# AHSAppDevTeam/Voxmap

Measured on AMD Instinct MI355X. Metric: Mrays/s at 3840x2160 full quality (C3); fps; % HBM roofline, higher is better.
Workload: dtype fp32

## Files before the change

voxmap_amd/csrc/vx_frame.cpp:

```cpp
#include <algorithm>
#include <cmath>
#include <cstring>

#include "vx_internal.h"

namespace vx {

static inline float gmax(float x, float y) { return x < y ? y : x; }
static inline float gmix(float x, float y, float a) { return x * (1.0f - a) + y * a; }
static inline float gsign(float x) { return x > 0.0f ? 1.0f : (x < 0.0f ? -1.0f : 0.0f); }

void sun_ray(const float r[3], SunRay &s) {
    for (int i = 0; i < 3; i++) {
        s.r[i] = r[i];
        s.sign[i] = gsign(r[i]);
        s.abs[i] = std::fabs(r[i]);
        s.rcp[i] = s.abs[i] != 0.0f ? 1.0f / s.abs[i] : 0.0f;
    }
    s.up = r[2] > 0.0f ? 1 : 0;
    const float lim = 0.0009765625f;
    s.fast = s.abs[0] >= lim && s.abs[1] >= lim && s.abs[2] >= lim;
}

static const double kVogel[VX_MAX_SHADOW_SAMPLES][2] = {
// ... 8 lines not shown
    {0.9393212963241181, 0.343038630874102},
    {-0.9243455561378048, 0.38155640847493627},
    {0.4238459950479107, -0.9057342725556136},
    {0.2992838644448729, 0.954164120307897},
    {-0.86521120975323, -0.5014075812324265},
    {0.976675773628176, -0.21471942904125782},
    {-0.5751294291397393, 0.8180624302199665},
    {-0.12851068979899324, -0.9917081236973845},
};

void sun_samples(const float sun[3], float radius, int n, float out[][3]) {
    if (n <= 1) {
        for (int i = 0; i < 3; i++) out[0][i] = sun[i];
        return;
    }
    n = n > VX_MAX_SHADOW_SAMPLES ? VX_MAX_SHADOW_SAMPLES : n;
    const double sd[3] = {sun[0], sun[1], sun[2]};
    const bool zax = std::fabs(sd[2]) < 0.9;
    const double ax[3] = {zax ? 0.0 : 1.0, 0.0, zax ? 1.0 : 0.0};
    double u[3] = {ax[1] * sd[2] - ax[2] * sd[1], ax[2] * sd[0] - ax[0] * sd[2], ax[0] * sd[1] - ax[1] * sd[0]};
    const double ul = std::sqrt(u[0] * u[0] + u[1] * u[1] + u[2] * u[2]);
    for (double &c : u) c /= ul;
    const double v[3] = {sd[1] * u[2] - sd[2] * u[1], sd[2] * u[0] - sd[0] * u[2], sd[0] * u[1] - sd[1] * u[0]};
    for (int k = 0; k < n; k++) {
        const double r = (double)radius * std::sqrt(((double)k + 0.5) / (double)n);
        const double cu = r * kVogel[k][0], cv = r * kVogel[k][1];
        double x[3];
        for (int i = 0; i < 3; i++) x[i] = sd[i] + cu * u[i] + cv * v[i];
        const double l = std::sqrt(x[0] * x[0] + x[1] * x[1] + x[2] * x[2]);
        for (int i = 0; i < 3; i++) out[k][i] = (float)(x[i] / l);
    }
}

void frame_consts(const vx_frame_params &p, int w, int h, int X, int Y, int Z, int max_steps, FrameConsts &fc) {
    std::memset(&fc, 0, sizeof fc);
    for (int i = 0; i < 3; i++) {
        fc.cam_cell[i] = p.cam_cell[i];
        fc.cam_fract[i] = p.cam_fract[i];
        fc.cam_cell_f[i] = (float)p.cam_cell[i];
        fc.fwd[i] = p.ray_fwd[i];
        fc.right[i] = p.ray_right[i];
        fc.up[i] = p.ray_up[i];
        fc.sun[i] = p.sun_dir[i];
        fc.sun_sign[i] = gsign(p.sun_dir[i]);
        fc.sun_abs[i] = std::fabs(p.sun_dir[i]);
        fc.sun_rcp[i] = fc.sun_abs[i] != 0.0f ? 1.0f / fc.sun_abs[i] : 0.0f;
        const int dim = i == 0 ? X : (i == 1 ? Y : Z);
        fc.slab_lo[i] = (float)(0 - p.cam_cell[i]) - p.cam_fract[i];
        fc.slab_hi[i] = (float)(dim - p.cam_cell[i]) - p.cam_fract[i];
        fc.cell_lo[i] = (float)(-p.cam_cell[i]);
        fc.cell_hi[i] = (float)(dim - p.cam_cell[i] - 1);
    }
    fc.fw = (float)w;
    fc.fh = (float)h;
    fc.rcp_w = 1.0f / fc.fw;
    fc.rcp_h = 1.0f / fc.fh;
    fc.sun_up = p.sun_dir[2] > 0.0f ? 1 : 0;
    const float lim = 0.0009765625f;
    fc.march_fast = fc.sun_abs[0] >= lim && fc.sun_abs[1] >= lim && fc.sun_abs[2] >= lim;
    fc.max_steps = max_steps;
    const float scatter = 1.0f - std::sqrt(gmax(0.0f, p.sun_dir[2]));
    const float sp0[3] = {0.2f, 0.4f, 0.7f}, sp1[3] = {0.2f, 0.3f, 0.5f};
    const float sc0[3] = {0.7f, 0.9f, 1.0f}, sc1[3] = {1.0f, 0.3f, 0.2f};
    for (int i = 0; i < 3; i++) {
        fc.spaceCol[i] = gmix(sp0[i], sp1[i], scatter);
        fc.scatterCol[i] = gmix(sc0[i], sc1[i], scatter);
        fc.shadeCol[i] = 0.7f * fc.scatterCol[i];
    }
// ... 84 lines not shown
```

voxmap_amd/csrc/vx_internal.h:

```cpp
#pragma once
#include <stddef.h>
#include <stdint.h>
#include <string>
#include <vector>
#include "../../include/voxmap.h"

namespace vx {

int set_error(int code, const std::string &msg);
const char *last_error();
int decode_container(const unsigned char *in, size_t n, int format, const char *key,
                     std::vector<unsigned char> &out, size_t expect);
int format_from_path(const char *path);
int encrypt_blob(const unsigned char *in, size_t n, const char *key, std::vector<unsigned char> &out);
int field_build(const uint8_t *color, int X, int Y, int Z, uint8_t *rgba, int n_threads);
int noise_synth(uint32_t seed, int w, int h, uint8_t *out);
int scene_device(const vx_scene *s);
void *scene_stream(const vx_scene *s);

struct SunRay {
    float r[3], sign[3], abs[3], rcp[3];
    int up;
    int fast;
};
void sun_ray(const float r[3], SunRay &s);
void sun_samples(const float sun[3], float radius, int n, float out[][3]);

struct FrameConsts {
    int cam_cell[3];
    float cam_fract[3];
    float cam_cell_f[3];
    float slab_lo[3], slab_hi[3], cell_lo[3], cell_hi[3];
    float fwd[3], right[3], up[3];
    float fw, fh, rcp_w, rcp_h;
    float sun[3];
    float sun_sign[3];
    float sun_abs[3], sun_rcp[3];
    int sun_up;
    int march_fast;
    int max_steps;
    float scatterCol[3], spaceCol[3], shadeCol[3];
    float shadeFactor[6];
    float normalCol[6][3];
    float sf[3];
    float cloudTime;
    float skyOff[2];
    int quality;
    unsigned flags;
    int n_sun;
    int soft_sg;
    int soft_lg;
    SunRay sun_k[VX_MAX_SHADOW_SAMPLES];
};

struct KernelArgs {
    const uint32_t *prim;
    const uint8_t *sun;
    const int8_t *sunp;
    int SB;
    float SBf;
    int SXp;
    unsigned SXpYp, sunp_texels;
    const int8_t *sunx;
    const int8_t *sunc;
    const uint16_t *rg;
    const uint32_t *rg2;
    const uint32_t *noise;
// ... 112 lines not shown
```

voxmap_amd/csrc/vx_render.h:

```cpp
#pragma once
#include <hip/hip_runtime.h>
#include <stdint.h>

#include "vx_internal.h"
#ifndef VX_QSPEC
#define VX_QSPEC 1
#endif

namespace vx {
namespace {

constexpr int kWG = 256;
constexpr int kGlass = 21;
constexpr float kInf = __builtin_inff();

__device__ __forceinline__ float gmin(float x, float y) { return y < x ? y : x; }
__device__ __forceinline__ float gmax(float x, float y) { return x < y ? y : x; }
__device__ __forceinline__ float gclamp(float x, float a, float b) { return gmin(gmax(x, a), b); }
__device__ __forceinline__ float gmix(float x, float y, float a) { return x * (1.0f - a) + y * a; }
__device__ __forceinline__ int f2i(float x) {
    const float c = __builtin_fminf(__builtin_fmaxf(x, -16777216.0f), 16777216.0f);
    const int r = (int)c;
    return x == x ? r : 0;
}

__device__ __forceinline__ float div_const(float a, float b, float y) {
    const float q0 = a * y;
    const float r0 = __builtin_fmaf(-q0, b, a);
    return __builtin_fmaf(r0, y, q0);
}

__device__ __forceinline__ float div_shared(float a, float b, float y) {
    return __builtin_copysignf(div_const(a, b, y), a);
}

__device__ __forceinline__ float rcp_ranged(float l) {
    const float r = __builtin_amdgcn_rcpf(l);
    return __builtin_fmaf(__builtin_fmaf(-l, r, 1.0f), r, r);
}


__device__ __forceinline__ float sqrt_ranged(float x) {
    const float s = __builtin_amdgcn_sqrtf(x);
    const float dn = __uint_as_float(__float_as_uint(s) - 1u), up = __uint_as_float(__float_as_uint(s) + 1u);
    float r = __builtin_fmaf(-dn, s, x) <= 0.0f ? dn : s;
    r = __builtin_fmaf(-up, s, x) > 0.0f ? up : r;
    return r;
}

__device__ __forceinline__ float vexp2(float x) {
    if (x != x) return x;
    if (x >= 128.0f) return kInf;
// ... 570 lines not shown
    const bool hit = stop != 0 && t < kSentinel;
    const int hax = tb0 == te ? 0 : (tb1 == te ? 1 : 2);
    int nrec = 0;
    const bool gl = gmark != kGlass;
    const bool gpos = gax == 0 ? p0 : (gax == 1 ? p1 : p2);
    const bool hpos = hax == 0 ? p0 : (hax == 1 ? p1 : p2);
    const float gr0 = g0h - hp0, gr1 = g1h - hp1, gr2 = g2h - hp2;
    const float hr0 = h0 - hp0, hr1 = h1 - hp1, hr2 = h2 - hp2;
    float gq0 = 0.0f, gq1 = 0.0f, gq2 = 0.0f, hq0 = 0.0f, hq1 = 0.0f, hq2 = 0.0f;
    if (a.quad_gbuf) {
        if (QSPEC) {
            if (__ballot(gl) != 0) qcopy_offsets(gqw, gax, gq0, gq1, gq2);
            qcopy_offsets(qw, hax, hq0, hq1, hq2);
        } else {
            if (gl) quad_offsets(a, gax, 2 * gax + (gpos ? 1 : 0), (int)gr0 + cc0, (int)gr1 + cc1, (int)gr2 + cc2, gq0, gq1, gq2);
            if (hit) quad_offsets(a, hax, 2 * hax + (hpos ? 1 : 0), (int)hr0 + cc0, (int)hr1 + cc1, (int)hr2 + cc2, hq0, hq1, hq2);
        }
    }
    if (gl) {
        const float upf = gpos ? 0.0f : 1.0f;
        const float r0 = gr0 - gq0, r1 = gr1 - gq1, r2 = gr2 - gq2;
        g0.id = 2;
        g0.color = kGlass;
        g0.nidx = 2 * gax + (gpos ? 1 : 0);
        g0.c0 = (r0 + F.cam_cell_f[0]) + (gax == 0 ? upf : 0.0f);
        g0.c1 = (r1 + F.cam_cell_f[1]) + (gax == 1 ? upf : 0.0f);
        g0.c2 = (r2 + F.cam_cell_f[2]) + (gax == 2 ? upf : 0.0f);
        g0.f0 = gax == 0 ? 0.0f : (o0 + gt * d0) - r0;
        g0.f1 = gax == 1 ? 0.0f : (o1 + gt * d1) - r1;
        g0.f2 = gax == 2 ? 0.0f : (o2 + gt * d2) - r2;
        nrec = 1;
    }
    if (hit) {
        Surf &h = gl ? g1 : g0;
        const float upf = hpos ? 0.0f : 1.0f;
        const float r0 = hr0 - hq0, r1 = hr1 - hq1, r2 = hr2 - hq2;
        h.id = col == kGlass ? 2 : 0;
        h.color = (int)col;
        h.nidx = 2 * hax + (hpos ? 1 : 0);
        h.c0 = (r0 + F.cam_cell_f[0]) + (hax == 0 ? upf : 0.0f);
        h.c1 = (r1 + F.cam_cell_f[1]) + (hax == 1 ? upf : 0.0f);
        h.c2 = (r2 + F.cam_cell_f[2]) + (hax == 2 ? upf : 0.0f);
        h.f0 = hax == 0 ? 0.0f : (o0 + te * d0) - r0;
        h.f1 = hax == 1 ? 0.0f : (o1 + te * d1) - r1;
        h.f2 = hax == 2 ? 0.0f : (o2 + te * d2) - r2;
        nrec++;
    }
    t_hit = te;
    return nrec;
}

__device__ __forceinline__ unsigned long long face_key(const KernelArgs &a, int x, int y, int z, int nidx,
                                                       unsigned q) {
    const int CH = a.chunk;
    const int d = nidx >> 1, normal = nidx & 1;
    const int cd_ = d == 0 ? x : (d == 1 ? y : z);
    const int cu = d == 0 ? y : (d == 1 ? z : x);
    const int cv = d == 0 ? z : (d == 1 ? x : y);
    const int plane = cd_ + (normal ? 0 : 1);
    int kd = plane / CH, pd = plane % CH - 1;
    if (pd < 0) { kd -= 1; pd = CH - 1; }
    const int ou = cu - (int)(q & 0xffu), ov = cv - (int)(q >> 8);
    const int ku = ou / CH, kv = ov / CH;
    const int kx = d == 0 ? kd : (d == 1 ? kv : ku);
    const int ky = d == 1 ? kd : (d == 2 ? kv : ku);
    const int kz = d == 2 ? kd : (d == 0 ? kv : ku);
    const unsigned long long ny = (unsigned long long)((a.Y + CH - 1) / CH), nz = (unsigned long long)((a.Z + CH - 1) / CH);
    const unsigned long long S = (unsigned long long)CH + 1;
    const unsigned long long chunk = ((unsigned long long)kx * ny + (unsigned long long)ky) * nz + (unsigned long long)kz;
    return ((((chunk * 3 + (unsigned long long)d) * 2 + (unsigned long long)normal) * S + (unsigned long long)(pd + 1)) * S +
            (unsigned long long)(ov - kv * CH)) * S + (unsigned long long)(ou - ku * CH);
}

__device__ __forceinline__ bool glass_scan(const KernelArgs &a, float d0, float d1, float d2, bool have_last,
                                           unsigned long long klast, float tmax, Surf &h, float &t_out,
                                           unsigned long long &k_out, bool &nearest) {
    const FrameConsts &F = a.fc;
    const float o0 = F.cam_fract[0], o1 = F.cam_fract[1], o2 = F.cam_fract[2];
// ... 101 lines not shown
    const int i = (int)fl;
    const int j = i + 1;
    i0 = min(max(i, 0), size - 1);
    i1 = min(max(j, 0), size - 1);
}

__device__ __forceinline__ float sdf_lin(const KernelArgs &a, float c0, float c1, float c2, float f0, float f1, float f2) {
    const FrameConsts &F = a.fc;
    int y0, y1, z0, z1;
    float wx, wy, wz;
    const float ux = (c0 + f0) * F.sf[0] * (float)a.X - 0.5f;
    const float flx = floorf(ux);
    wx = ux - flx;
    const int px = min(max((int)flx, -1), a.X - 1) + 1;
    lin_axis((c1 + f1) * F.sf[1], a.Y, y0, y1, wy);
    lin_axis((c2 + f2) * F.sf[2], a.Z, z0, z1, wz);
    const unsigned row = (unsigned)a.X + 1u;
    const unsigned b00 = ((unsigned)px + __umul24(row, (unsigned)y0) + __umul24(__umul24(row, (unsigned)a.Y), (unsigned)z0)) << 2;
    const unsigned dy = __umul24((unsigned)(y1 - y0), 4u * row), dz = __umul24((unsigned)(z1 - z0), 4u * row * (unsigned)a.Y);
    const u32x4 rs = buf_rsrc(a.rg2, kRsrcRGBA);
    const f32x4 u00 = ld_fmt4(rs, b00), u10 = ld_fmt4(rs, b00 + dy);
    const f32x4 u01 = ld_fmt4(rs, b00 + dz), u11 = ld_fmt4(rs, b00 + dy + dz);
    float res[2];
#pragma unroll
    for (int ch = 0; ch < 2; ch++) {
        const float v00 = gmix(u00[ch], u00[2 + ch], wx);
        const float v01 = gmix(u10[ch], u10[2 + ch], wx);
        const float v10 = gmix(u01[ch], u01[2 + ch], wx);
        const float v11 = gmix(u11[ch], u11[2 + ch], wx);
        const float w0 = gmix(v00, v01, wy);
        const float w1 = gmix(v10, v11, wy);
        res[ch] = gmix(w0, w1, wz) * 255.0f;
    }
    return gmin(res[0], res[1]);
}

__device__ __forceinline__ int wrap_idx(float fl, int n) {
    int r = (int)fl & (n - 1);
    if (!(fabsf(fl) < 16777216.0f)) {
        const float q = floorf(fl * (1.0f / (float)n));
        r = f2i(fl - q * (float)n) & (n - 1);
    }
    return r;
}

__device__ __forceinline__ float fbm(const KernelArgs &a, float px, float py) {
    const int W = a.noise_w, H = a.noise_h;
    const float u = px * (float)W - 0.5f, v = py * (float)H - 0.5f;
    const float fu = floorf(u), fv = floorf(v);
    const float wa = u - fu, wb = v - fv;
    const int x0 = wrap_idx(fu, W), y0 = wrap_idx(fv, H);
    const u32x4 rs = buf_rsrc(a.noise4, kRsrcRGBA);
    const f32x4 t = ld_fmt4(rs, (((unsigned)y0 << a.noise_lw) | (unsigned)x0) << 2);
    const float r0 = gmix(t.x, t.y, wa), r1 = gmix(t.z, t.w, wa);
    return 1.0f - 2.0f * gmix(r0, r1, wb);
}

__device__ __forceinline__ void normalize3_ranged(float v0, float v1, float v2, float &o0, float &o1, float &o2) {
    const float l = sqrt_ranged(v0 * v0 + v1 * v1 + v2 * v2);
    const float y = rcp_ranged(l);
    o0 = div_shared(v0, l, y); o1 = div_shared(v1, l, y); o2 = div_shared(v2, l, y);
}
__device__ __forceinline__ void normalize3(float v0, float v1, float v2, float &o0, float &o1, float &o2) {
    const float l = sqrtf(v0 * v0 + v1 * v1 + v2 * v2);
    const float y = 1.0f / l;
    o0 = div_shared(v0, l, y); o1 = div_shared(v1, l, y); o2 = div_shared(v2, l, y);
}

__device__ __forceinline__ void shade_sky(const KernelArgs &a, float d0, float d1, float d2, float o[4],
                          Counters &cnt) {
    const FrameConsts &F = a.fc;
    float r0, r1, r2;
    normalize3(d0, d1, d2, r0, r1, r2);
    const float k = 2.0f * ((-1.0f * r0 + 0.0f * r1) + 0.0f * r2);
    const float refl_z = r2 - k * 0.0f;
    const float sunCol[3] = {1.4f, 1.0f, 0.5f};
    float sunFactor = gmax(0.0f, F.sun[0] * r0 + F.sun[1] * r1 + F.sun[2] * r2) - 1.0f;
    const float glow = vexp2(8.0f * sunFactor);
    sunFactor = vexp2(4000.0f * sunFactor) + 0.3f * glow;
    const float rz = sqrtf(gmax(0.0f, refl_z));
    float sky[3];
#pragma unroll
    for (int i = 0; i < 3; i++) {
        const float atm = gmix(F.scatterCol[i], F.spaceCol[i], rz);
        sky[i] = gclamp(sunCol[i] * sunFactor + atm, 0.0f, 1.0f);
    }
    r2 = fabsf(r2);
    if (F.flags & VX_FLAG_NO_CLOUDS) {
        o[0] = sky[0]; o[1] = sky[1]; o[2] = sky[2]; o[3] = 1.0f;
        return;
    }
    cnt.noise_px++;
    const float ct = F.cloudTime;
    const float den = sqrt_ranged(fabsf(r2) + 0.03f);
    float sx, sy;
    {
        const float y = rcp_ranged(den);
        sx = div_shared(r0, den, y); sy = div_shared(r1, den, y);
    }
    sx = sx * 0.1f; sy = sy * 0.1f;
    const float sl = sqrtf(sqrtf(sx * sx + sy * sy));
    sx = sx * sl; sy = sy * sl;
    const float n0 = fbm(a, 2.0f * sx + ct, 2.0f * sy + ct);
    const float n1 = fbm(a, 2.0f * sx - ct, 2.0f * sy - ct);
    const float mountainPos = r0 / r1;
    float mountainHeight = 1.0f - fbm(a, 0.3f * mountainPos, 0.3f * mountainPos);
    mountainHeight = mountainHeight / (vexp(0.3f * mountainPos * mountainPos) * 6.0f);
    if (mountainHeight > r2 && r1 > 0.0f && r2 > 0.0f) {
        const float mountainFactor = 2.0f - fbm(a, 2.0f * (mountainPos + r1), 2.0f * (mountainPos + r2));
        const float mt[3] = {0.7f, 0.8f, 0.7f};
        const float w = mountainFactor * r2;
#pragma unroll
        for (int i = 0; i < 3; i++) sky[i] = gmix(sky[i], sky[i] * mt[i], w);
    } else {
        sx = sx * (3.0f + n0); sy = sy * (3.0f + n1);
        sx = sx + F.skyOff[0];
        sy = sy + F.skyOff[1];
        const float cloudFactor = vexp2(6.0f * (fbm(a, sx + 2.0f * ct, sy + -9.0f * ct) - 1.0f));
        const float scf = sqrtf(cloudFactor);
#pragma unroll
        for (int i = 0; i < 3; i++) sky[i] = gmix(sky[i], gmix(sunCol[i], 0.8f, scf), cloudFactor);
    }
    o[0] = sky[0]; o[1] = sky[1]; o[2] = sky[2]; o[3] = 1.0f;
}

__device__ __forceinline__ void white(const KernelArgs &a, float px, float py, float &w0, float &w1, float &w2) {
    const int W = a.noise_w, H = a.noise_h;
    const float u = px * (float)W - 0.5f, v = py * (float)H - 0.5f;
    const float fu = floorf(u), fv = floorf(v);
    const float wa = u - fu, wb = v - fv;
    const int x0 = wrap_idx(fu, W), y0 = wrap_idx(fv, H);
    const unsigned off = (((unsigned)y0 << a.noise_lw) | (unsigned)x0) << 2, plane = ((unsigned)W * (unsigned)H) << 2;
    const u32x4 rs = buf_rsrc(a.noise4, kRsrcRGBA);
    const f32x4 tr = ld_fmt4(rs, off + plane), tg = ld_fmt4(rs, off + 2u * plane), tb = ld_fmt4(rs, off + 3u * plane);
    auto bil = [&](const f32x4 &t) { return 1.0f - 2.0f * gmix(gmix(t.x, t.y, wa), gmix(t.z, t.w, wa), wb); };
    w0 = bil(tr); w1 = bil(tg); w2 = bil(tb);
}

constexpr float kRoughScale = 0.00390625f;
constexpr float kRoughAmp = 0.1f;

template <int EXT>
__device__ __forceinline__ float block_shade_factor(const KernelArgs &a, const Surf &g) {
    const FrameConsts &F = a.fc;
    const int ni = g.nidx;
    if (!(EXT && (F.flags & VX_FLAG_ROUGH))) return F.shadeFactor[ni];
    const float n0 = ni == 0 ? 1.0f : (ni == 1 ? -1.0f : 0.0f);
    const float n1 = ni == 2 ? 1.0f : (ni == 3 ? -1.0f : 0.0f);
    const float n2 = ni == 4 ? 1.0f : (ni == 5 ? -1.0f : 0.0f);
    const int ax = ni >> 1;
    const float u = ax == 0 ? g.c1 + g.f1 : g.c0 + g.f0;
    const float v = ax == 2 ? g.c1 + g.f1 : g.c2 + g.f2;
    float w0, w1, w2, m0, m1, m2;
    white(a, u * kRoughScale, v * kRoughScale, w0, w1, w2);
    normalize3_ranged(n0 + kRoughAmp * w0, n1 + kRoughAmp * w1, n2 + kRoughAmp * w2, m0, m1, m2);
    return F.sun[2] < 0.0f ? 0.0f : sqrtf(gmax(0.0f, (m0 * F.sun[0] + m1 * F.sun[1]) + m2 * F.sun[2]));
}

template <int EXT>
__device__ __forceinline__ void shade_block(const KernelArgs &a, const Surf &g, float o[4], Counters &cnt,
                            bool has_ray = false, float q0 = 0.0f, float q1 = 0.0f, float q2 = 0.0f,
                            float *ray_out = nullptr, int lit_given = -1) {
    const FrameConsts &F = a.fc;
    const int ni = g.nidx;
    const float n0 = ni == 0 ? 1.0f : (ni == 1 ? -1.0f : 0.0f);
    const float n1 = ni == 2 ? 1.0f : (ni == 3 ? -1.0f : 0.0f);
    const float n2 = ni == 4 ? 1.0f : (ni == 5 ? -1.0f : 0.0f);
    float r0, r1, r2;
    if (EXT && has_ray) {
        r0 = q0; r1 = q1; r2 = q2;
    } else {
        normalize3((g.c0 - F.cam_cell_f[0]) + (g.f0 - F.cam_fract[0]),
                   (g.c1 - F.cam_cell_f[1]) + (g.f1 - F.cam_fract[1]),
                   (g.c2 - F.cam_cell_f[2]) + (g.f2 - F.cam_fract[2]), r0, r1, r2);
    }
    if (EXT && ray_out) { ray_out[0] = r0; ray_out[1] = r1; ray_out[2] = r2; }
    float m0 = n0, m1 = n1, m2 = n2;
    const bool rough = EXT && (F.flags & VX_FLAG_ROUGH);
    if (rough) {
        cnt.rough++;
        const int ax = ni >> 1;
        const float u = ax == 0 ? g.c1 + g.f1 : g.c0 + g.f0;
        const float v = ax == 2 ? g.c1 + g.f1 : g.c2 + g.f2;
        float w0, w1, w2;
        white(a, u * kRoughScale, v * kRoughScale, w0, w1, w2);
        normalize3_ranged(n0 + kRoughAmp * w0, n1 + kRoughAmp * w1, n2 + kRoughAmp * w2, m0, m1, m2);
    }
    float base0 = 1.0f, base1 = 1.0f, base2 = 1.0f;
    if (g.color < 22) { base0 = kPalette[g.color][0]; base1 = kPalette[g.color][1]; base2 = kPalette[g.color][2]; }
    float amb0 = 1.0f, amb1 = 1.0f, amb2 = 1.0f;
    if (!(F.flags & VX_FLAG_NO_AO)) {
        cnt.ao++;
        const float ambDist = sdf_lin(a, g.c0 + n0, g.c1 + n1, g.c2 + n2, g.f0, g.f1, g.f2);
        const float ambFactor = gmin(1.0f - sqrtf(ambDist), 0.8f);
        amb0 = gmix(1.0f, F.shadeCol[0], ambFactor);
        amb1 = gmix(1.0f, F.shadeCol[1], ambFactor);
        amb2 = gmix(1.0f, F.shadeCol[2], ambFactor);
    }
    float shadeFactor = F.shadeFactor[ni];
    if (rough)
        shadeFactor = F.sun[2] < 0.0f ? 0.0f : sqrtf(gmax(0.0f, (m0 * F.sun[0] + m1 * F.sun[1]) + m2 * F.sun[2]));
    if (shadeFactor > 0.0f && !(F.flags & VX_FLAG_NO_SHADOW)) {
        const int sg0 = sun_sg(F.sun_k[0]);
        const int8_t *xch = EXT != 2 || !a.sunp || !F.sun_k[0].fast ? nullptr
                          : a.sunc ? a.sunc
                          : a.sunx && F.soft_sg >= 0 ? a.sunx + (size_t)sg0 * a.sunp_texels : nullptr;
        const bool first_exit = xch && lit_given < 0 && first_step_exit(a, xch, sg0, g);
        if (EXT != 2) {
            cnt.shadow_rays++;
            const bool lit = march_sun(a, F.sun_k[0], g.c0, g.c1, g.c2, g.f0, g.f1, g.f2, cnt);
            shadeFactor = shadeFactor * (lit ? 1.0f : 0.0f);
        } else if (lit_given >= 0) {
            shadeFactor = shadeFactor * ((float)lit_given / (float)F.n_sun);
        } else if (first_exit) {
            cnt.shadow_rays += (unsigned)F.n_sun;
            cnt.shadow_resolved += (unsigned)F.n_sun;
        } else {
            int lit = 0;
            if (xch) {
                switch (sg0) {
#define VX_SGS(K) case K: lit = march_soft<K>(a, xch, g.c0, g.c1, g.c2, g.f0, g.f1, g.f2, cnt); break;
                    VX_SGS(0) VX_SGS(1) VX_SGS(2) VX_SGS(3) VX_SGS(4) VX_SGS(5) VX_SGS(6)
                    default: lit = march_soft<7>(a, xch, g.c0, g.c1, g.c2, g.f0, g.f1, g.f2, cnt);
#undef VX_SGS
                }
            } else {
                for (int k = 0; k < F.n_sun; k++) {
// ... 124 lines not shown
    unsigned long long klast = 0;
    bool have_last = false, nearest = false;
    Surf cur;
    float tc;
    unsigned long long kc;
    while (glass_scan(a, d0, d1, d2, have_last, klast, depth, cur, tc, kc, nearest) && !nearest) {
        depth = tc; klast = kc; have_last = true;
        float src[4], rd[3];
        shade_block<XE>(a, cur, src, cnt, false, 0.0f, 0.0f, 0.0f, rd);
        if (XE && (F.flags & (VX_FLAG_REFLECT | VX_FLAG_REFLECT_ALL))) {
            float refl[3];
            reflect_color<XE>(a, cur, rd, refl, cnt);
            const int ax = cur.nidx >> 1;
            const float cs = gmin(fabsf(ax == 0 ? rd[0] : (ax == 1 ? rd[1] : rd[2])), 1.0f);
            const float x = 1.0f - cs, x2 = x * x;
            const float fr = 0.04f + 0.96f * ((x2 * x2) * x);
#pragma unroll
            for (int i = 0; i < 3; i++) src[i] = src[i] + fr * refl[i];
        }
        blend_canvas(src, dst, dst);
    }
}

__device__ __forceinline__ unsigned long long wave_sum(unsigned v) {
    unsigned long long s = v;
#pragma unroll
    for (int off = 32; off > 0; off >>= 1) s += __shfl_xor(s, off, 64);
    return s;
}

__device__ __forceinline__ uint32_t pack_rgba8(const float rgba[4]) {
    uint32_t pk = 0;
#pragma unroll
    for (int i = 0; i < 4; i++) pk |= (uint32_t)(gclamp(rgba[i], 0.0f, 1.0f) * 255.0f + 0.5f) << (8 * i);
    return pk;
}

template <int FMT>
__device__ __forceinline__ void store_pixel(const KernelArgs &a, size_t idx, const float rgba[4]) {
    if (FMT == VX_PIXEL_RGBA32F)
        reinterpret_cast<float4 *>(a.out)[idx] = make_float4(rgba[0], rgba[1], rgba[2], rgba[3]);
    else
        reinterpret_cast<uint32_t *>(a.out)[idx] = pack_rgba8(rgba);
}

template <bool TILED>
__device__ __forceinline__ size_t out_index(const KernelArgs &a, int k, int x, int y, int px, int py) {
    if (TILED && !a.tile_inplace) return (size_t)k * a.tile_h * a.tile_pitch + (size_t)y * a.tile_pitch + x;
    return (size_t)py * a.w + px;
}

__device__ __forceinline__ void view_ray(const FrameConsts &F, int px, int py, float &d0, float &d1, float &d2) {
    const float nx = div_const((float)(2 * px + 1), F.fw, F.rcp_w) - 1.0f;
    const float ny = 1.0f - div_const((float)(2 * py + 1), F.fh, F.rcp_h);
    d0 = (F.fwd[0] + nx * F.right[0]) + ny * F.up[0];
    d1 = (F.fwd[1] + nx * F.right[1]) + ny * F.up[1];
    d2 = (F.fwd[2] + nx * F.right[2]) + ny * F.up[2];
}

__device__ __forceinline__ void primary_only_colour(int n, const Surf &g0, float rgba[4]) {
    const int pc = n == 0 ? 0 : g0.color;
    rgba[0] = pc < 22 ? kPalette[pc][0] : 1.0f;
    rgba[1] = pc < 22 ? kPalette[pc][1] : 1.0f;
    rgba[2] = pc < 22 ? kPalette[pc][2] : 1.0f;
    rgba[3] = 1.0f;
}

constexpr float kClear2d = 0.9f;
__device__ __forceinline__ void shade_2d(const KernelArgs &a, float d0, float d1, float d2, float rgba[4], Counters &cnt,
                         unsigned &n_sky, unsigned &n_block, unsigned &n_glass) {
    const FrameConsts &F = a.fc;
    rgba[0] = rgba[1] = rgba[2] = kClear2d;
    rgba[3] = 1.0f;
    const float zr = (float)(0 - F.cam_cell[2]) - F.cam_fract[2];
    int c = 0, x = 0, y = 0;
    float hx = 0.0f, hy = 0.0f;
// ... 191 lines not shown
                                               cnt); break;
                                VX_SGB(0) VX_SGB(1) VX_SGB(2) VX_SGB(3) VX_SGB(4) VX_SGB(5) VX_SGB(6)
                                default: lit = march_brick<7>(a, S, ch, br, ox, oy, oz, pc.x, pc.y, pc.z, pf.x, pf.y,
                                                              pf.z, cnt);
#undef VX_SGB
                            }
                        } else {
                            switch (sgv) {
#define VX_SGP(K) case K: lit = march_pad<K, kDoomAfter>(a, S, ch, pc.x, pc.y, pc.z, pf.x, pf.y, pf.z, \
                                                   cnt); break;
                                VX_SGP(0) VX_SGP(1) VX_SGP(2) VX_SGP(3) VX_SGP(4) VX_SGP(5) VX_SGP(6)
                                default: lit = march_pad<7, kDoomAfter>(a, S, ch, pc.x, pc.y, pc.z, pf.x, pf.y, pf.z,
                                                                  cnt);
#undef VX_SGP
                            }
                        }
                        if (lit) atomicAdd(&s_plit[wb + fs], 1);
                    }
                }
                __builtin_amdgcn_fence(__ATOMIC_ACQUIRE, "wavefront");
                __builtin_amdgcn_wave_barrier();
                if (need) lit0 = s_plit[wb + slot];
            }
        }
        if (!kPool || inframe) {
            float rgba[4];
            if (F.flags & VX_FLAG_PRIMARY_ONLY) {
                primary_only_colour(n, g[0], rgba);
                n_sky = n == 0;
                n_glass = n != 0 && g[0].id == 2;
                n_block = n != 0 && g[0].id != 2;
            } else if (n == 0) {
                n_sky = 1;
                shade_sky(a, d0, d1, d2, rgba, cnt);
            } else {
if constexpr (!kGeneral) {
                float dst[4];
                if (g[0].id == 2) {
                    if (n == 2) shade_block<XE>(a, g[1], dst, cnt);
                    else shade_sky(a, d0, d1, d2, dst, cnt);
                    if (__builtin_expect(__ballot(stacked) != 0, 0) && stacked)
                        glass_chain<XE>(a, d0, d1, d2, dst, n == 2 ? t_hit : kInf, cnt);
                }
                float rd[3];
                shade_block<XE>(a, g[0], rgba, cnt, false, 0.0f, 0.0f, 0.0f, rd, lit0);
                if (g[0].id == 2) {
                    n_glass = 1;
                    if (XE && (F.flags & VX_FLAG_REFLECT)) {
                        float refl[3];
                        reflect_color<XE>(a, g[0], rd, refl, cnt);
                        const int ax = g[0].nidx >> 1;
                        const float cs = gmin(fabsf(ax == 0 ? rd[0] : (ax == 1 ? rd[1] : rd[2])), 1.0f);
                        const float x = 1.0f - cs, x2 = x * x;
                        const float fr = 0.04f + 0.96f * ((x2 * x2) * x);
#pragma unroll
                        for (int i = 0; i < 3; i++) rgba[i] = rgba[i] + fr * refl[i];
                    }
                    blend_canvas(rgba, dst, rgba);
                } else {
                    n_block = 1;
                }
                (void)t_hit;
} else {
                float dst[4];
                const bool glass = g[0].id == 2;
                if (glass) {
                    if (n == 2) shade_block<XE>(a, g[1], dst, cnt);
                    else shade_sky(a, d0, d1, d2, dst, cnt);
                    if (__builtin_expect(__ballot(stacked) != 0, 0) && stacked)
                        glass_chain<XE>(a, d0, d1, d2, dst, n == 2 ? t_hit : kInf, cnt);
                }
                float rd[3];
                shade_block<XE>(a, g[0], rgba, cnt, false, 0.0f, 0.0f, 0.0f, rd, lit0);
                if (XE && (F.flags & (glass ? (VX_FLAG_REFLECT | VX_FLAG_REFLECT_ALL) : VX_FLAG_REFLECT_ALL))) {
                    float refl[3];
                    reflect_color<XE>(a, g[0], rd, refl, cnt);
                    const int ax = g[0].nidx >> 1;
                    const float cs = gmin(fabsf(ax == 0 ? rd[0] : (ax == 1 ? rd[1] : rd[2])), 1.0f);
                    const float x = 1.0f - cs, x2 = x * x;
                    const float fr = 0.04f + 0.96f * ((x2 * x2) * x);
#pragma unroll
                    for (int i = 0; i < 3; i++) rgba[i] = rgba[i] + fr * refl[i];
                }
                if (glass) {
                    n_glass = 1;
                    blend_canvas(rgba, dst, rgba);
                } else {
                    n_block = 1;
                }
}
            }
            rgba[3] = 1.0f;
            store_pixel<FMT>(a, TILED ? (size_t)toidx : out_index<TILED>(a, tile_k, tx0 + lx, ty0 + ly, px, py), rgba);
            n_px = 1;
        }
    }
#ifdef VX_BLOCK_TIMING
    __syncthreads();
    if (threadIdx.x == 0 && a.blk_time) {
        const size_t b = (size_t)blockIdx.x + (size_t)blockIdx.y * gridDim.x;
        a.blk_time[2 * b] = t_blk0;
        a.blk_time[2 * b + 1] = __builtin_amdgcn_s_memrealtime();
    }
#endif
    if (STATS) {
        unsigned long long v[ST_COUNT];
        v[ST_PIXELS] = wave_sum(n_px);
        v[ST_SKY] = wave_sum(n_sky);
        v[ST_BLOCK] = wave_sum(n_block);
        v[ST_GLASS] = wave_sum(n_glass);
        v[ST_PRIM_FETCH] = wave_sum(cnt.prim_fetch);
        v[ST_SHADOW_RAYS] = wave_sum(cnt.shadow_rays);
        v[ST_SHADOW_FETCH] = wave_sum(cnt.shadow_fetch);
        v[ST_AO] = wave_sum(cnt.ao);
        v[ST_NOISE_PX] = wave_sum(cnt.noise_px);
        v[ST_CAP_HITS] = wave_sum(cnt.cap_hit);
        v[ST_REFL_RAYS] = wave_sum(cnt.refl_rays);
        v[ST_REFL_FETCH] = wave_sum(cnt.refl_fetch);
        v[ST_ROUGH] = wave_sum(cnt.rough);
        v[ST_PRIM_WITERS] = wave_sum(cnt.prim_witers);
        v[ST_MARCH_WITERS] = wave_sum(cnt.march_witers);
        v[ST_MARCH_SLOTS] = wave_sum(cnt.march_slots);
        v[ST_SHADOW_RESOLVED] = wave_sum(cnt.shadow_resolved);
        if (lane == 0) {
            unsigned long long *row = a.stats + (size_t)((blockIdx.x + blockIdx.y * 7) & 63) * ST_COUNT;
#pragma unroll
// ... 45 lines not shown
```

voxmap_amd/kernel_meta.py:

```python
from __future__ import annotations

import os
import re
import subprocess
import tempfile

LLVM = "/opt/rocm/lib/llvm/bin"
TARGET = "hipv4-amdgcn-amd-amdhsa--gfx950"
FIELDS = ("private_segment_fixed_size", "vgpr_count", "sgpr_count", "vgpr_spill_count", "sgpr_spill_count",
          "group_segment_fixed_size")
RENDER_SCRATCH_LIMIT = 256
STATS_SCRATCH_LIMIT = 0
STATS_SPILL_LIMIT = 0
HOT_LOOP_SPILL_LIMITS = {1: 8, 2: 2, 5: 8}
SPILL_LIMITS = {0: 19, 1: 62, 2: 64, 3: 70, 4: 132, 5: 16, 6: 16}
V1_SCRATCH_LIMIT = 72
RENDER_VGPR_LIMIT = 64
GENERAL_VGPR_LIMIT = 96


def _tool(name: str) -> str:
    p = os.path.join(LLVM, name)
    return p if os.path.exists(p) else name

# ... 11 lines not shown
        with open(part, "wb") as f:
            f.write(data[s:starts[i + 1] if i + 1 < len(starts) else len(data)])
        subprocess.run([_tool("clang-offload-bundler"), "--unbundle", "--type=o", f"--targets={TARGET}",
                        f"--input={part}", f"--output={co}"], check=True, capture_output=True)
        out.append(co)
    return out


def kernels(lib: str) -> dict[str, dict[str, int]]:
    notes = ""
    with tempfile.TemporaryDirectory() as d:
        for co in code_objects(lib, d):
            notes += subprocess.run([_tool("llvm-readelf"), "--notes", co], check=True, capture_output=True,
                                    text=True).stdout
    out: dict[str, dict[str, int]] = {}
    blocks, cur = [], None
    for line in notes.splitlines():
        if re.match(r"\s+- \.", line):
            cur = {}
            blocks.append(cur)
        if cur is None:
            continue
        m = re.match(r"\s+(?:- )?\.name:\s+(\S+)$", line)
        if m:
            cur["__name"] = m.group(1)
            continue
        m = re.match(r"\s+(?:- )?\.(\w+):\s+(\d+)$", line)
        if m and m.group(1) in FIELDS:
            cur[m.group(1)] = int(m.group(2))
    for b in blocks:
        name = b.pop("__name", None)
        if name and "private_segment_fixed_size" in b:
            out[name] = b
    return out


def render_params(name: str):
    m = re.search(r"k_render(?:_gen)?ILi(\d)ELb(\d)ELb(\d)ELi(\d)ELb(\d)E", name)
    return tuple(int(g) for g in m.groups()) if m else None


def hot_loop_spills(lib: str, ext_max: int = 6) -> dict[tuple, tuple[int, int]]:
    out: dict[tuple, tuple[int, int]] = {}
    with tempfile.TemporaryDirectory() as d:
        for co in code_objects(lib, d):
            txt = subprocess.run([_tool("llvm-objdump"), "-d", "--no-show-raw-insn", co], check=True,
                                 capture_output=True, text=True).stdout
            name, body = None, []
            for line in txt.splitlines() + ["0 <END>:"]:
                m = re.match(r"^[0-9a-f]+ <(.+)>:$", line)
                if m:
                    p = render_params(name) if name else None
                    if p and p[0] == 1 and p[1] == 0 and p[3] <= ext_max:
                        out[p] = _hot_spills(body)
                    name, body = m.group(1), []
                elif name and "//" in line:
                    ins, cmt = line.split("//", 1)
                    am = re.match(r"\s*([0-9A-Fa-f]+):", cmt)
                    if am:
                        body.append((int(am.group(1), 16), ins.strip()))
    return out


def _hot_spills(body: list[tuple[int, str]]) -> tuple[int, int]:
    end = next((i for i, (_, l) in enumerate(body) if l.startswith("s_endpgm")), len(body))
    body = body[:end]
# ... 9 lines not shown
        off = off - 65536 if off >= 32768 else off
        tgt = index.get(a + 4 + 4 * off)
        if tgt is not None and tgt < i:
            back.append((tgt, i))
    loops = n = 0
    for h, e in back:
        if (e - h > 400 or any(h <= h2 and e2 <= e and (h2, e2) != (h, e) for h2, e2 in back)
                or not any(hot[h:e + 1])):
            continue
        loops += 1
        n = max(n, sum(spill[h:e + 1]))
    return loops, n


def check(lib: str) -> dict[str, dict[str, int]]:
    ks = kernels(lib)
    render = {k: v for k, v in ks.items() if "k_render" in k}
    if not render:
        raise RuntimeError(f"{lib}: no k_render kernels found in the gfx950 code object")
    bad = []
    for name, v in render.items():
        p = render_params(name)
        stats = p is not None and p[1] == 1
        brick = p is not None and p[3] == 4
        lim = STATS_SCRATCH_LIMIT if stats else RENDER_SCRATCH_LIMIT
        if v.get("private_segment_fixed_size", 0) > lim:
            bad.append(f"{name}: private segment {v['private_segment_fixed_size']} B > {lim}")
        spill_lim = STATS_SPILL_LIMIT if stats else SPILL_LIMITS.get(p[3]) if p is not None else None
        if spill_lim is not None and v.get("vgpr_spill_count", 0) > spill_lim:
            bad.append(f"{name}: {v['vgpr_spill_count']} VGPRs spilled > {spill_lim}")
        general = p is not None and p[3] >= 5
        if not stats and v.get("vgpr_count", 0) > (80 if brick else GENERAL_VGPR_LIMIT if general else RENDER_VGPR_LIMIT):
            bad.append(f"{name}: {v['vgpr_count']} VGPRs > {RENDER_VGPR_LIMIT}")
    for p, (loops, n) in hot_loop_spills(lib).items():
        if not loops:
            bad.append(f"k_render{p}: no march / primary loop found in the disassembly (check the parser)")
        if n > HOT_LOOP_SPILL_LIMITS.get(p[3] if p else -1, 0):
            bad.append(f"k_render{p}: {n} spill instructions inside a march / primary loop")
    if bad:
        raise RuntimeError("render kernel resource check failed:\n  " + "\n  ".join(bad))
    return ks


if __name__ == "__main__":
    import sys
    lib = sys.argv[1] if len(sys.argv) > 1 else os.path.join(os.path.dirname(__file__), "libvoxmap_hip.so")
    for name, v in sorted(kernels(lib).items()):
        print(f"{name[:70]:70s} " + " ".join(f"{f.split('_')[0][:5]}={v.get(f, 0)}" for f in FIELDS))
```

Measured before the change: 131,000.

## Micro-optimize shading: med3 clamps, ranged sky normalize, uniform hit store, direct RGBA8 store

Bundles several small instruction-level changes in the render kernel. Clamps become fmed3 (relying on DX10 clamp mode), min becomes fminf, and axis normals are built by bit tricks. A host-side check lets the sky path use a cheaper ranged normalize when the camera basis is well conditioned. A wave-uniform ballot avoids select-heavy writes to the hit record when no lane hit glass, and the non-tiled RGBA8 store uses 32-bit offset math. A descriptor check is added to the resource validator. Each change trims a few ALU ops, in exchange for more code paths and reliance on hardware clamp semantics.

```diff
diff --git a/voxmap_amd/csrc/vx_frame.cpp b/voxmap_amd/csrc/vx_frame.cpp
--- a/voxmap_amd/csrc/vx_frame.cpp
+++ b/voxmap_amd/csrc/vx_frame.cpp
@@ -64,8 +64,21 @@
     }
 }
 
+static int rays_ranged(const vx_frame_params &p) {
+    const double f[3] = {p.ray_fwd[0], p.ray_fwd[1], p.ray_fwd[2]};
+    const double r[3] = {p.ray_right[0], p.ray_right[1], p.ray_right[2]};
+    const double u[3] = {p.ray_up[0], p.ray_up[1], p.ray_up[2]};
+    auto len = [](const double v[3]) { return std::sqrt(v[0] * v[0] + v[1] * v[1] + v[2] * v[2]); };
+    const double n[3] = {r[1] * u[2] - r[2] * u[1], r[2] * u[0] - r[0] * u[2], r[0] * u[1] - r[1] * u[0]};
+    const double S = len(f) + len(r) + len(u), ln = len(n);
+    if (!(ln > 0.0) || !(S < 0x1p40) || !(S >= 0x1p-28)) return 0;
+    const double dist = std::fabs(f[0] * n[0] + f[1] * n[1] + f[2] * n[2]) / ln;
+    return dist >= S * 0x1p-10 ? 1 : 0;
+}
+
 void frame_consts(const vx_frame_params &p, int w, int h, int X, int Y, int Z, int max_steps, FrameConsts &fc) {
     std::memset(&fc, 0, sizeof fc);
+    fc.rays_ranged = rays_ranged(p);
     for (int i = 0; i < 3; i++) {
         fc.cam_cell[i] = p.cam_cell[i];
         fc.cam_fract[i] = p.cam_fract[i];
diff --git a/voxmap_amd/csrc/vx_internal.h b/voxmap_amd/csrc/vx_internal.h
--- a/voxmap_amd/csrc/vx_internal.h
+++ b/voxmap_amd/csrc/vx_internal.h
@@ -33,6 +33,7 @@
     float slab_lo[3], slab_hi[3], cell_lo[3], cell_hi[3];
     float fwd[3], right[3], up[3];
     float fw, fh, rcp_w, rcp_h;
+    int rays_ranged;
     float sun[3];
     float sun_sign[3];
     float sun_abs[3], sun_rcp[3];
diff --git a/voxmap_amd/csrc/vx_render.h b/voxmap_amd/csrc/vx_render.h
--- a/voxmap_amd/csrc/vx_render.h
+++ b/voxmap_amd/csrc/vx_render.h
@@ -18,6 +18,9 @@
 __device__ __forceinline__ float gmax(float x, float y) { return x < y ? y : x; }
 __device__ __forceinline__ float gclamp(float x, float a, float b) { return gmin(gmax(x, a), b); }
 __device__ __forceinline__ float gmix(float x, float y, float a) { return x * (1.0f - a) + y * a; }
+__device__ __forceinline__ float fmin_fin(float x, float y) { return __builtin_fminf(x, y); }
+__device__ __forceinline__ float fmax_fin(float x, float y) { return __builtin_fmaxf(x, y); }
+__device__ __forceinline__ float clamp01(float x) { return __builtin_amdgcn_fmed3f(x, 0.0f, 1.0f); }
 __device__ __forceinline__ int f2i(float x) {
     const float c = __builtin_fminf(__builtin_fmaxf(x, -16777216.0f), 16777216.0f);
     const int r = (int)c;
@@ -654,18 +657,28 @@
         nrec = 1;
     }
     if (hit) {
-        Surf &h = gl ? g1 : g0;
         const float upf = hpos ? 0.0f : 1.0f;
         const float r0 = hr0 - hq0, r1 = hr1 - hq1, r2 = hr2 - hq2;
-        h.id = col == kGlass ? 2 : 0;
-        h.color = (int)col;
-        h.nidx = 2 * hax + (hpos ? 1 : 0);
-        h.c0 = (r0 + F.cam_cell_f[0]) + (hax == 0 ? upf : 0.0f);
-        h.c1 = (r1 + F.cam_cell_f[1]) + (hax == 1 ? upf : 0.0f);
-        h.c2 = (r2 + F.cam_cell_f[2]) + (hax == 2 ? upf : 0.0f);
-        h.f0 = hax == 0 ? 0.0f : (o0 + te * d0) - r0;
-        h.f1 = hax == 1 ? 0.0f : (o1 + te * d1) - r1;
-        h.f2 = hax == 2 ? 0.0f : (o2 + te * d2) - r2;
+        const int id = col == kGlass ? 2 : 0;
+        const int nidx = 2 * hax + (hpos ? 1 : 0);
+        const float c0 = (r0 + F.cam_cell_f[0]) + (hax == 0 ? upf : 0.0f);
+        const float c1 = (r1 + F.cam_cell_f[1]) + (hax == 1 ? upf : 0.0f);
+        const float c2 = (r2 + F.cam_cell_f[2]) + (hax == 2 ? upf : 0.0f);
+        const float f0 = hax == 0 ? 0.0f : (o0 + te * d0) - r0;
+        const float f1 = hax == 1 ? 0.0f : (o1 + te * d1) - r1;
+        const float f2 = hax == 2 ? 0.0f : (o2 + te * d2) - r2;
+        if (__builtin_expect(__ballot(gl) == 0, 1)) {
+            g0.id = id; g0.color = (int)col; g0.nidx = nidx;
+            g0.c0 = c0; g0.c1 = c1; g0.c2 = c2;
+            g0.f0 = f0; g0.f1 = f1; g0.f2 = f2;
+        } else {
+            g1.id = id; g1.color = (int)col; g1.nidx = nidx;
+            g1.c0 = c0; g1.c1 = c1; g1.c2 = c2;
+            g1.f0 = f0; g1.f1 = f1; g1.f2 = f2;
+            g0.id = gl ? g0.id : id; g0.color = gl ? g0.color : (int)col; g0.nidx = gl ? g0.nidx : nidx;
+            g0.c0 = gl ? g0.c0 : c0; g0.c1 = gl ? g0.c1 : c1; g0.c2 = gl ? g0.c2 : c2;
+            g0.f0 = gl ? g0.f0 : f0; g0.f1 = gl ? g0.f1 : f1; g0.f2 = gl ? g0.f2 : f2;
+        }
         nrec++;
     }
     t_hit = te;
@@ -833,7 +846,7 @@
         const float w1 = gmix(v10, v11, wy);
         res[ch] = gmix(w0, w1, wz) * 255.0f;
     }
-    return gmin(res[0], res[1]);
+    return fmin_fin(res[0], res[1]);
 }
 
 __device__ __forceinline__ int wrap_idx(float fl, int n) {
@@ -868,11 +881,11 @@
     o0 = div_shared(v0, l, y); o1 = div_shared(v1, l, y); o2 = div_shared(v2, l, y);
 }
 
-__device__ __forceinline__ void shade_sky(const KernelArgs &a, float d0, float d1, float d2, float o[4],
-                          Counters &cnt) {
-    const FrameConsts &F = a.fc;
-    float r0, r1, r2;
-    normalize3(d0, d1, d2, r0, r1, r2);
+template <bool RANGED>
+__device__ __forceinline__ void sky_clear(const FrameConsts &F, float d0, float d1, float d2, float &r0, float &r1,
+                                          float &r2, float sky[3]) {
+    if (RANGED) normalize3_ranged(d0, d1, d2, r0, r1, r2);
+    else normalize3(d0, d1, d2, r0, r1, r2);
     const float k = 2.0f * ((-1.0f * r0 + 0.0f * r1) + 0.0f * r2);
     const float refl_z = r2 - k * 0.0f;
     const float sunCol[3] = {1.4f, 1.0f, 0.5f};
@@ -880,12 +893,22 @@
     const float glow = vexp2(8.0f * sunFactor);
     sunFactor = vexp2(4000.0f * sunFactor) + 0.3f * glow;
     const float rz = sqrtf(gmax(0.0f, refl_z));
-    float sky[3];
 #pragma unroll
     for (int i = 0; i < 3; i++) {
         const float atm = gmix(F.scatterCol[i], F.spaceCol[i], rz);
-        sky[i] = gclamp(sunCol[i] * sunFactor + atm, 0.0f, 1.0f);
-    }
+        const float v = sunCol[i] * sunFactor + atm;
+        sky[i] = RANGED ? clamp01(v) : gclamp(v, 0.0f, 1.0f);
+    }
+}
+
+__device__ __forceinline__ void shade_sky(const KernelArgs &a, float d0, float d1, float d2, float o[4],
+                          Counters &cnt, bool ranged = false) {
+    const FrameConsts &F = a.fc;
+    const float sunCol[3] = {1.4f, 1.0f, 0.5f};
+    float r0, r1, r2;
+    float sky[3];
+    if (ranged) sky_clear<true>(F, d0, d1, d2, r0, r1, r2, sky);
+    else sky_clear<false>(F, d0, d1, d2, r0, r1, r2, sky);
     r2 = fabsf(r2);
     if (F.flags & VX_FLAG_NO_CLOUDS) {
         o[0] = sky[0]; o[1] = sky[1]; o[2] = sky[2]; o[3] = 1.0f;
@@ -941,14 +964,21 @@
 constexpr float kRoughScale = 0.00390625f;
 constexpr float kRoughAmp = 0.1f;
 
+__device__ __forceinline__ void axis_normal(int ni, float &n0, float &n1, float &n2) {
+    const float s = __uint_as_float(0x3f800000u | ((unsigned)ni << 31));
+    const int ax = ni >> 1;
+    n0 = ax == 0 ? s : 0.0f;
+    n1 = ax == 1 ? s : 0.0f;
+    n2 = ax == 2 ? s : 0.0f;
+}
+
 template <int EXT>
 __device__ __forceinline__ float block_shade_factor(const KernelArgs &a, const Surf &g) {
     const FrameConsts &F = a.fc;
     const int ni = g.nidx;
     if (!(EXT && (F.flags & VX_FLAG_ROUGH))) return F.shadeFactor[ni];
-    const float n0 = ni == 0 ? 1.0f : (ni == 1 ? -1.0f : 0.0f);
-    const float n1 = ni == 2 ? 1.0f : (ni == 3 ? -1.0f : 0.0f);
-    const float n2 = ni == 4 ? 1.0f : (ni == 5 ? -1.0f : 0.0f);
+    float n0, n1, n2;
+    axis_normal(ni, n0, n1, n2);
     const int ax = ni >> 1;
     const float u = ax == 0 ? g.c1 + g.f1 : g.c0 + g.f0;
     const float v = ax == 2 ? g.c1 + g.f1 : g.c2 + g.f2;
@@ -964,9 +994,8 @@
                             float *ray_out = nullptr, int lit_given = -1) {
     const FrameConsts &F = a.fc;
     const int ni = g.nidx;
-    const float n0 = ni == 0 ? 1.0f : (ni == 1 ? -1.0f : 0.0f);
-    const float n1 = ni == 2 ? 1.0f : (ni == 3 ? -1.0f : 0.0f);
-    const float n2 = ni == 4 ? 1.0f : (ni == 5 ? -1.0f : 0.0f);
+    float n0, n1, n2;
+    axis_normal(ni, n0, n1, n2);
     float r0, r1, r2;
     if (EXT && has_ray) {
         r0 = q0; r1 = q1; r2 = q2;
@@ -993,7 +1022,7 @@
     if (!(F.flags & VX_FLAG_NO_AO)) {
         cnt.ao++;
         const float ambDist = sdf_lin(a, g.c0 + n0, g.c1 + n1, g.c2 + n2, g.f0, g.f1, g.f2);
-        const float ambFactor = gmin(1.0f - sqrtf(ambDist), 0.8f);
+        const float ambFactor = fmin_fin(1.0f - sqrt_ranged(ambDist), 0.8f);
         amb0 = gmix(1.0f, F.shadeCol[0], ambFactor);
         amb1 = gmix(1.0f, F.shadeCol[1], ambFactor);
         amb2 = gmix(1.0f, F.shadeCol[2], ambFactor);
@@ -1184,7 +1213,7 @@
 __device__ __forceinline__ uint32_t pack_rgba8(const float rgba[4]) {
     uint32_t pk = 0;
 #pragma unroll
-    for (int i = 0; i < 4; i++) pk |= (uint32_t)(gclamp(rgba[i], 0.0f, 1.0f) * 255.0f + 0.5f) << (8 * i);
+    for (int i = 0; i < 4; i++) pk |= (uint32_t)(clamp01(rgba[i]) * 255.0f + 0.5f) << (8 * i);
     return pk;
 }
 
@@ -1194,6 +1223,10 @@
         reinterpret_cast<float4 *>(a.out)[idx] = make_float4(rgba[0], rgba[1], rgba[2], rgba[3]);
     else
         reinterpret_cast<uint32_t *>(a.out)[idx] = pack_rgba8(rgba);
+}
+__device__ __forceinline__ void store_rgba8_frame(const KernelArgs &a, int px, int py, const float rgba[4]) {
+    const unsigned off = ((unsigned)py * (unsigned)a.w + (unsigned)px) << 2;
+    *reinterpret_cast<uint32_t *>(reinterpret_cast<char *>(a.out) + off) = pack_rgba8(rgba);
 }
 
 template <bool TILED>
@@ -1451,7 +1484,7 @@
                 n_block = n != 0 && g[0].id != 2;
             } else if (n == 0) {
                 n_sky = 1;
-                shade_sky(a, d0, d1, d2, rgba, cnt);
+                shade_sky(a, d0, d1, d2, rgba, cnt, F.rays_ranged != 0);
             } else {
 if constexpr (!kGeneral) {
                 float dst[4];
@@ -1510,7 +1543,10 @@
 }
             }
             rgba[3] = 1.0f;
-            store_pixel<FMT>(a, TILED ? (size_t)toidx : out_index<TILED>(a, tile_k, tx0 + lx, ty0 + ly, px, py), rgba);
+            if constexpr (!TILED && FMT == VX_PIXEL_RGBA8)
+                store_rgba8_frame(a, px, py, rgba);
+            else
+                store_pixel<FMT>(a, TILED ? (size_t)toidx : out_index<TILED>(a, tile_k, tx0 + lx, ty0 + ly, px, py), rgba);
             n_px = 1;
         }
     }
diff --git a/voxmap_amd/kernel_meta.py b/voxmap_amd/kernel_meta.py
--- a/voxmap_amd/kernel_meta.py
+++ b/voxmap_amd/kernel_meta.py
@@ -67,6 +67,24 @@
         name = b.pop("__name", None)
         if name and "private_segment_fixed_size" in b:
             out[name] = b
+    return out
+
+
+def descriptor_modes(lib: str) -> dict[str, dict[str, int]]:
+    out: dict[str, dict[str, int]] = {}
+    with tempfile.TemporaryDirectory() as d:
+        for co in code_objects(lib, d):
+            txt = subprocess.run([_tool("llvm-objdump"), "-d", "-j", ".rodata", co], check=True,
+                                 capture_output=True, text=True).stdout
+            cur = None
+            for line in txt.splitlines():
+                m = re.match(r"\.amdhsa_kernel\s+(\S+)", line)
+                if m:
+                    cur = out.setdefault(m.group(1), {})
+                    continue
+                m = re.match(r"\s+\.amdhsa_(dx10_clamp|ieee_mode)\s+(\d+)", line)
+                if m and cur is not None:
+                    cur[m.group(1)] = int(m.group(2))
     return out
 
 
@@ -142,6 +160,10 @@
         general = p is not None and p[3] >= 5
         if not stats and v.get("vgpr_count", 0) > (80 if brick else GENERAL_VGPR_LIMIT if general else RENDER_VGPR_LIMIT):
             bad.append(f"{name}: {v['vgpr_count']} VGPRs > {RENDER_VGPR_LIMIT}")
+    modes = descriptor_modes(lib)
+    for name in render:
+        if modes.get(name, {}).get("dx10_clamp") != 1:
+            bad.append(f"{name}: DX10_CLAMP is not set in the kernel descriptor ({modes.get(name)})")
     for p, (loops, n) in hot_loop_spills(lib).items():
         if not loops:
             bad.append(f"k_render{p}: no march / primary loop found in the disassembly (check the parser)")
```

After: 135,600, median of 6. 1.03x the previous value.
